# LiuTaowen-Tony/xKV

Measured on NVIDIA B200. Metric: KV GB/s compressed (prefill, xKV-4, Llama-3.1-8B 64K), higher is better.
Workload: dtype bf16

## Files before the change

include/xkv_b200.h:

```cpp
#ifndef XKV_B200_H_
#define XKV_B200_H_

#include <stddef.h>
#include <stdint.h>

#ifdef __cplusplus
extern "C" {
#endif

#if defined(__GNUC__)
#define XKV_API __attribute__((visibility("default")))
#else
#define XKV_API
#endif

#define XKV_MAX_GROUP_LAYERS 16
#define XKV_MAX_GEMM_PROBLEMS 16
#define XKV_MAX_BATCH 16
#define XKV_MAX_LAYER_MAPS 64

XKV_API const char* xkv_last_error(void);
XKV_API int xkv_version(void);
XKV_API int64_t xkv_launch_count(void);

XKV_API int xkv_pack_group(const void* const* layer_ptrs_host, int num_layers, int bs, int heads, int seq,
                   int head_dim, int64_t stride_b, int64_t stride_h, int64_t stride_s, void* X,
                   void* stream);
XKV_API int xkv_unpack_group(const void* X, int num_layers, int bs, int heads, int seq, int head_dim,
                     int64_t stride_b, int64_t stride_h, int64_t stride_s, void* const* layer_ptrs_host,
                     void* stream);

typedef struct xkv_gemm_problem {
  int32_t M, N, K;
  int32_t num_terms;
  int32_t a_mn_major;
  int32_t b_mn_major;
  const void* A[3];
  const void* B[3];
  int64_t lda, ldb;
  uint8_t term_a[6], term_b[6];
  void* D;
  int64_t ldd;
  int32_t out_bf16;
  int32_t out_transposed;
  int32_t sym_upper;
  int32_t split_k;
  int64_t split_stride;
  int32_t accum_phases;
  const int32_t* run_if;
  int32_t a_layers, b_layers, layer_cols;
  const void* A_layer[XKV_MAX_GROUP_LAYERS];
  const void* B_layer[XKV_MAX_GROUP_LAYERS];
} xkv_gemm_problem;
XKV_API int xkv_gemm_grouped(const xkv_gemm_problem* problems_host, int num_problems, void* stream);
XKV_API size_t xkv_gemm_problem_size(void);
XKV_API void xkv_gemm_set_gram_pair(int on);

XKV_API int xkv_reduce_slabs(const float* slabs, int num_slabs, int64_t slab_stride, int rows, int cols, int64_t ld,
                     int symmetrize, float* out, int64_t ld_out, void* stream);
XKV_API int xkv_reduce_slabs_batched(const float* const* slabs_host, float* const* out_host, int batch, int num_slabs,
                                     int64_t slab_stride, int rows, int cols, int64_t ld, int symmetrize,
                                     int64_t ld_out, void* stream);
XKV_API int xkv_split_bf16(const float* x, int rows, int cols, int64_t ld, void* hi, void* mid, void* lo,
                   int64_t ld_out, void* stream);
XKV_API int xkv_split_bf16_batched(const float* const* x_host, void* const* hi_host, void* const* mid_host,
                                   void* const* lo_host, int batch, int rows, int cols, int64_t ld, int64_t ld_out,
                                   void* stream);
XKV_API int xkv_symmetrize_split_bf16(const float* const* slabs_host, int batch, int num_slabs, int64_t slab_stride,
                                      int n, int64_t ld, void* const* hi_host, void* const* mid_host,
                                      void* const* lo_host, int64_t ld_out, void* stream);
XKV_API size_t xkv_gram_packed_elems(int n);
XKV_API int xkv_gram_pack_upper(const float* full, int n, int64_t ld, float* packed, void* stream);
XKV_API int xkv_gram_unpack_upper(const float* packed, int n, float* full, int64_t ld, void* stream);
XKV_API int xkv_fill_gaussian_bf16(void* out, int rows, int cols, int64_t ld, uint64_t seed, void* stream);
XKV_API int xkv_normalize_rows(float* const* Y_host, void* const* hi_host, void* const* mid_host,
                               void* const* lo_host, int batch, int rows, int cols, int64_t ld, int64_t ld_out,
                               void* stream);
XKV_API int xkv_shift_normalize_rows(float* const* Y_host, const float* const* Q_host, float* shift_dev,
                                     float* const* rdiag_host, int rdiag_first, void* const* hi_host,
                                     void* const* mid_host, void* const* lo_host, int batch, int rows, int cols,
                                     int64_t ld, int64_t ld_out, void* stream);
XKV_API int xkv_ritz_shift_update(float* const* rdiag_host, int batch, int rows, int tail_rows, float shift_scale,
                                  float* shift_dev, void* stream);
XKV_API int xkv_rdiag_update(float* const* rdiag_host, const float* const* Linv_host, int batch, int rows,
                             int64_t ld_linv, void* stream);
XKV_API int xkv_pass_flags(const float* const* Linv_host, int batch, int rows, int64_t ld_linv, float min_pivot,
                           int32_t* flags_dev, void* stream);
XKV_API void xkv_set_launch_predicate(const int32_t* flags_dev);
XKV_API int xkv_cholesky_inverse(float* const* S_host, float* const* Linv_host, int batch, int l, int64_t ld,
                                 float shift, float pivot_floor, void* stream);
XKV_API int xkv_cholesky_inverse_limbs(float* const* S_host, float* const* Linv_host, void* const* hi_host,
                                       void* const* mid_host, void* const* lo_host, int batch, int l, int64_t ld,
                                       int64_t ld_limb, float shift, float pivot_floor, void* stream);
XKV_API int xkv_jacobi_eigh(const float* const* T_host, float* const* evals_host, float* const* Wt_host, int count,
                            int W, int64_t ld, int64_t ld_w, int sweeps, void* stream);
XKV_API int xkv_convert_bf16(const float* src, int rows, int cols, int64_t ld, void* dst, int64_t ld_dst, void* dstT,
                             int64_t ld_dstT, void* stream);

XKV_API int xkv_sqrt_clamp(const float* in, float* out, int count, void* stream);

#define XKV_FACTORIZE_SIGMA_COUNT 128
// ... 62 lines not shown
```

xkv_b200/_lib.py:

```python
from __future__ import annotations

import ctypes as C
import os
from typing import Optional

_LIB_PATH = os.environ.get("XKV_B200_LIB") or os.path.join(os.path.dirname(os.path.abspath(__file__)), "libxkv_b200.so")
_lib: Optional[C.CDLL] = None

MAX_GROUP_LAYERS = 16
MAX_GEMM_PROBLEMS = 16
MAX_BATCH = 16
FACTORIZE_SIGMA_COUNT = 128


class XkvError(RuntimeError):
    """Raised when a C-ABI call returns a non-zero status (mirrors the reference's Python exceptions)."""


class GemmProblem(C.Structure):

    _fields_ = [
        ("M", C.c_int32),
        ("N", C.c_int32),
        ("K", C.c_int32),
        ("num_terms", C.c_int32),
        ("a_mn_major", C.c_int32),
        ("b_mn_major", C.c_int32),
        ("A", C.c_void_p * 3),
        ("B", C.c_void_p * 3),
        ("lda", C.c_int64),
        ("ldb", C.c_int64),
        ("term_a", C.c_uint8 * 6),
        ("term_b", C.c_uint8 * 6),
        ("D", C.c_void_p),
        ("ldd", C.c_int64),
        ("out_bf16", C.c_int32),
        ("out_transposed", C.c_int32),
        ("sym_upper", C.c_int32),
        ("split_k", C.c_int32),
        ("split_stride", C.c_int64),
        ("accum_phases", C.c_int32),
        ("run_if", C.c_void_p),
        ("a_layers", C.c_int32),
        ("b_layers", C.c_int32),
        ("layer_cols", C.c_int32),
        ("A_layer", C.c_void_p * MAX_GROUP_LAYERS),
        ("B_layer", C.c_void_p * MAX_GROUP_LAYERS),
    ]


class AppendProblem(C.Structure):

    _fields_ = [("x_new", C.c_void_p), ("V", C.c_void_p), ("a_out", C.c_void_p), ("ldx", C.c_int64), ("ldv", C.c_int64),
                ("lda", C.c_int64), ("n", C.c_int32), ("r", C.c_int32)]


_vp, _i, _i64, _f, _sz = C.c_void_p, C.c_int, C.c_int64, C.c_float, C.c_size_t
_pp = C.POINTER(C.c_void_p)
SIGNATURES = {
    "xkv_last_error": (C.c_char_p, []),
    "xkv_version": (_i, []),
    "xkv_launch_count": (_i64, []),
    "xkv_pack_group": (_i, [_pp, _i, _i, _i, _i, _i, _i64, _i64, _i64, _vp, _vp]),
    "xkv_unpack_group": (_i, [_vp, _i, _i, _i, _i, _i, _i64, _i64, _i64, _pp, _vp]),
    "xkv_gemm_grouped": (_i, [C.POINTER(GemmProblem), _i, _vp]),
    "xkv_reduce_slabs": (_i, [_vp, _i, _i64, _i, _i, _i64, _i, _vp, _i64, _vp]),
    "xkv_reduce_slabs_batched": (_i, [_pp, _pp, _i, _i, _i64, _i, _i, _i64, _i, _i64, _vp]),
    "xkv_symmetrize_split_bf16": (_i, [_pp, _i, _i, _i64, _i, _i64, _pp, _pp, _pp, _i64, _vp]),
    "xkv_split_bf16_batched": (_i, [_pp, _pp, _pp, _pp, _i, _i, _i, _i64, _i64, _vp]),
    "xkv_split_bf16": (_i, [_vp, _i, _i, _i64, _vp, _vp, _vp, _i64, _vp]),
    "xkv_gram_packed_elems": (_sz, [_i]),
    "xkv_gram_pack_upper": (_i, [_vp, _i, _i64, _vp, _vp]),
    "xkv_gram_unpack_upper": (_i, [_vp, _i, _vp, _i64, _vp]),
    "xkv_fill_gaussian_bf16": (_i, [_vp, _i, _i, _i64, C.c_uint64, _vp]),
    "xkv_normalize_rows": (_i, [_pp, _pp, _pp, _pp, _i, _i, _i, _i64, _i64, _vp]),
    "xkv_shift_normalize_rows": (_i, [_pp, _pp, _vp, _pp, _i, _pp, _pp, _pp, _i, _i, _i, _i64, _i64, _vp]),
    "xkv_ritz_shift_update": (_i, [_pp, _i, _i, _i, _f, _vp, _vp]),
    "xkv_rdiag_update": (_i, [_pp, _pp, _i, _i, _i64, _vp]),
    "xkv_pass_flags": (_i, [_pp, _i, _i, _i64, C.c_float, _vp, _vp]),
    "xkv_set_launch_predicate": (None, [_vp]),
    "xkv_cholesky_inverse": (_i, [_pp, _pp, _i, _i, _i64, _f, _f, _vp]),
    "xkv_cholesky_inverse_limbs": (_i, [_pp, _pp, _pp, _pp, _pp, _i, _i, _i64, _i64, _f, _f, _vp]),
    "xkv_jacobi_eigh": (_i, [_pp, _pp, _pp, _i, _i, _i64, _i64, _i, _vp]),
    "xkv_convert_bf16": (_i, [_vp, _i, _i, _i64, _vp, _i64, _vp, _i64, _vp]),
    "xkv_sqrt_clamp": (_i, [_vp, _vp, _i, _vp]),
    "xkv_factorize_workspace_bytes": (_sz, [_i, _i, _i, _i]),
    "xkv_decode_workspace_bytes": (_sz, [_i, _i, _i, _i]),
    "xkv_decode_attention": (_i, [_vp, _i, _i, _i, _vp, _i64, _i, _vp, _i64, _vp, _i64, _i, _vp, _i64, _i, _vp, _vp, _i64,
                                  _vp, _vp, _i, _i64, _i64, _f, _vp, _vp, _sz, _vp]),
    "xkv_decode_attention_lse": (_i, [_vp, _i, _i, _i, _vp, _i64, _i, _vp, _i64, _vp, _i64, _i, _vp, _i64, _i, _vp, _vp,
                                      _i64, _vp, _vp, _i, _i64, _i64, _f, _vp, _vp, _sz, _vp, _vp]),
    "xkv_decode_attention_multi": (_i, [_vp, _i, _i, _i, _i, _vp, _i64, _i, _vp, _i64, _vp, _i64, _i, _vp, _i64, _i, _vp,
                                        _vp, _i64, _vp, _vp, _i, _i64, _i64, _f, _vp, _vp, _sz, _vp, _vp]),
    "xkv_decode_absorbed_workspace_bytes": (_sz, [_i, _i, _i]),
# ... 43 lines not shown
```

xkv_b200/csrc/xkv_factorize.cu:

```cuda
#include <cuda_bf16.h>

#include <vector>

#include "xkv_host.h"

namespace xkv {

static inline size_t align_up(size_t x, size_t a) { return (x + a - 1) / a * a; }
static inline int round_up_int(int x, int k) { return (x + k - 1) / k * k; }

struct Bump {
  char* base;
  size_t off, cap;
  bool overflow;
  void* take(size_t bytes) {
    off = align_up(off, 1024);
    void* p = base ? base + off : nullptr;
    off += bytes;
    if (base && off > cap) overflow = true;
    return p;
  }
  float* f32(size_t n) { return static_cast<float*>(take(n * 4)); }
  void* bf16(size_t n) { return take(n * 2); }
};
// ... 252 lines not shown
    }
  }
  XKV_TRY(mark());
  if (phase == 1) return 0;

  float** cur = P.f_a;
  float** nxt = P.f_b;
  auto swap_bufs = [&]() {
    float** t = cur;
    cur = nxt;
    nxt = t;
  };
  auto cholqr = [&](bool shifted, bool track, bool final_call) -> int {
    const int first = shifted ? 1 : 0;
    for (int pp = first; pp <= first + 1; ++pp) {
      const bool cond = shifted && pp == 2;
      if (cond) {
        XKV_TRY(xkv_pass_flags(P.linv, B, l, l, kSecondPassMinPivot, P.pass_flags, stream));
        xkv_set_launch_predicate(P.pass_flags);
      }
      int rc = [&]() -> int {
        XKV_TRY(xkv_shift_normalize_rows(cur, (pp == first && shifted) ? nxt : nullptr, P.shift_dev,
                                         track ? P.rdiag : nullptr, pp == first, P.lh, P.lm, P.ll, B, l, n, nn, nn, stream));
        for (int b = 0; b < B; ++b) {
          xkv_gemm_problem p = problem(P.lh[b], P.lm[b], P.ll[b], nn, 0, P.lh[b], P.lm[b], P.ll[b], nn, 0, P.s_slabs[b],
                                       l, l, l, n, 6);
          p.sym_upper = 1;
          p.split_k = P.sk;
          p.split_stride = static_cast<long long>(l) * l;
          p.run_if = cond ? P.pass_flags + b : nullptr;
          ps.push_back(p);
        }
        XKV_TRY(run_gemms(ps, stream));
        XKV_TRY(xkv_reduce_slabs_batched(P.s_slabs, P.s_mat, B, P.sk, static_cast<long long>(l) * l, l, l, l, 1, l, stream));
        {
          void *h0[XKV_MAX_BATCH], *h1[XKV_MAX_BATCH], *h2[XKV_MAX_BATCH];
          for (int b = 0; b < B; ++b) h0[b] = P.linv_l[b][0], h1[b] = P.linv_l[b][1], h2[b] = P.linv_l[b][2];
          const float shift = kCholShift[pp];
          XKV_TRY(xkv_cholesky_inverse_limbs(P.s_mat, P.linv, h0, h1, h2, B, l, l, l, shift, kPivotFloor, stream));
          if (pp > 0) {
            XKV_TRY(xkv_pass_flags(P.linv, B, l, l, 2.f * shift, P.redo_flags, stream));
            xkv_set_launch_predicate(P.redo_flags);
            int rc2 = xkv_reduce_slabs_batched(P.s_slabs, P.s_mat, B, P.sk, static_cast<long long>(l) * l, l, l, l, 1, l, stream);
            if (!rc2)
              rc2 = xkv_cholesky_inverse_limbs(P.s_mat, P.linv, h0, h1, h2, B, l, l, l, kCholShift[0], kPivotFloor, stream);
            xkv_set_launch_predicate(cond ? P.pass_flags : nullptr);
            if (rc2) return rc2;
          }
        }
        if (track) XKV_TRY(xkv_rdiag_update(P.rdiag, P.linv, B, l, l, stream));
        for (int b = 0; b < B; ++b) {
          xkv_gemm_problem p = swap_roles(problem(P.linv_l[b][0], P.linv_l[b][1], P.linv_l[b][2], l, 0, P.lh[b], P.lm[b],
                                                  P.ll[b], nn, 1, cond ? cur[b] : nxt[b], nn, l, n, l, final_call ? 6 : 3));
          p.run_if = cond ? P.pass_flags + b : nullptr;
          ps.push_back(p);
        }
        XKV_TRY(run_gemms(ps, stream));
        return 0;
      }();
      if (cond) xkv_set_launch_predicate(nullptr);
      if (rc) return rc;
      if (!cond) swap_bufs();
    }
    return 0;
  };
  auto apply_gram = [&](int nterms) -> int {
    for (int b = 0; b < B; ++b)
      ps.push_back(swap_roles(problem(P.lh[b], P.lm[b], P.ll[b], nn, 0, P.g_limb[b][0], P.g_limb[b][1], P.g_limb[b][2], nn, 0,
                                      nxt[b], nn, l, n, n, nterms)));
    XKV_TRY(run_gemms(ps, stream));
    swap_bufs();
    return 0;
  };

  for (int b = 0; b < B; ++b) XKV_TRY(xkv_fill_gaussian_bf16(P.lh[b], l, n, nn, kSeed + 7919ull * b, stream));
  XKV_TRY(apply_gram(1));
  XKV_TRY(cholqr(false, false, false));
  XKV_TRY(mark());

  XKV_CHECK_CUDA(cudaMemsetAsync(P.shift_dev, 0, XKV_MAX_BATCH * sizeof(float), st));
  for (int it = 0; it < kPowerSteps; ++it) {
    XKV_TRY(xkv_split_bf16_batched(cur, P.lh, P.lm, nullptr, B, l, n, nn, nn, stream));
    XKV_TRY(apply_gram(3));
    if (it > 0) XKV_TRY(xkv_ritz_shift_update(P.rdiag, B, l, kShiftTail, kSpectralShift, P.shift_dev, stream));
    const bool last = it == kPowerSteps - 1;
    XKV_TRY(cholqr(it > 0, !last, last));
  }
  XKV_TRY(mark());

  {
    const int r0 = l - W, wl = r - r0;
    auto w0 = [&](int w) { return w == 0 ? r0 : 0; };
    XKV_TRY(xkv_split_bf16_batched(cur, P.lh, P.lm, P.ll, B, l, n, nn, nn, stream));
    for (int b = 0; b < B; ++b)
      for (int w = 0; w < 2; ++w)
        ps.push_back(swap_roles(problem(row_bf16(P.lh[b], w0(w), nn), row_bf16(P.lm[b], w0(w), nn),
                                        row_bf16(P.ll[b], w0(w), nn), nn, 0, P.g_limb[b][0], P.g_limb[b][1], P.g_limb[b][2],
                                        nn, 0, P.yw[b][w], nn, W, n, n, 6)));
    XKV_TRY(run_gemms(ps, stream));
    {
      const float* xs[2 * XKV_MAX_BATCH];
      void *h0[2 * XKV_MAX_BATCH], *h1[2 * XKV_MAX_BATCH], *h2[2 * XKV_MAX_BATCH];
      int cntw = 0;
      for (int b = 0; b < B; ++b)
        for (int w = 0; w < 2; ++w) {
          xs[cntw] = P.yw[b][w];
// ... 89 lines not shown
```

xkv_b200/csrc/xkv_gemm.cu:

```cuda
#include <cstdlib>

#include "xkv_common.cuh"
#include "xkv_host.h"

namespace xkv {

constexpr int BM = 128;
constexpr int BN = 256;
constexpr int BK = 64;
constexpr int STAGES = 4;
constexpr int A_TILE_BYTES = BM * BK * 2;
constexpr int B_TILE_BYTES = BN * BK * 2;
constexpr int STAGE_BYTES = A_TILE_BYTES + B_TILE_BYTES;
constexpr int CHUNK_BYTES = 64 * BK * 2;
constexpr int GEMM_THREADS = 192;
constexpr int TMEM_COLS = 256;
constexpr size_t GEMM_SMEM_BYTES = STAGES * STAGE_BYTES + 1024  + 256 ;

struct alignas(64) GemmProb {
  CUtensorMap a_map[3];
  CUtensorMap b_map[3];
  void* D;
  long long ldd;
  long long split_stride;
  int M, N, K;
  int nterms;
  int tiles_m, tiles_n, ntiles;
  int split_k, kblocks_per_split, nkb;
  int cta_begin;
  int bn;
  int na, nb;
  unsigned char la[3], lb[3];
  unsigned char sa[3], sb[3];
  int pstages;
  int out_bf16, out_transposed, sym_upper;
  unsigned char ta[6], tb[6];
  const int* run_if;
  int phases;
  int a_layers, a_layer_begin, b_layers, b_layer_begin, layer_cols;
};
struct GemmParams {
  int nprob;
  int pair_stages;
  GemmProb p[XKV_MAX_GEMM_PROBLEMS];
  CUtensorMap layer_maps[XKV_MAX_LAYER_MAPS];
};

__device__ __forceinline__ const CUtensorMap* layer_map(const GemmParams& P, int begin, int layers, int layer_cols, int col,
                                                        int& col_in_layer) {
  int li = col / layer_cols;
  li = li < layers ? li : layers - 1;
  col_in_layer = col - li * layer_cols;
  return &P.layer_maps[begin + li];
}

template <int A_MN, int B_MN>
__global__ void __launch_bounds__(GEMM_THREADS, 1) gemm_kernel(const __grid_constant__ GemmParams P) {
  extern __shared__ uint8_t smem_raw[];
  uint8_t* smem = reinterpret_cast<uint8_t*>((reinterpret_cast<uintptr_t>(smem_raw) + 1023) & ~uintptr_t(1023));
  uint64_t* full_bar = reinterpret_cast<uint64_t*>(smem + STAGES * STAGE_BYTES);
  uint64_t* empty_bar = full_bar + STAGES;
  uint64_t* tmem_full_bar = empty_bar + STAGES;
  uint64_t* tmem_empty_bar = tmem_full_bar + 2;
  uint32_t* tmem_slot = reinterpret_cast<uint32_t*>(tmem_empty_bar + 2);

  const int warp = threadIdx.x >> 5;
  const int lane = threadIdx.x & 31;

  int pi = 0;
  while (pi + 1 < P.nprob && static_cast<int>(blockIdx.x) >= P.p[pi + 1].cta_begin) ++pi;
  const GemmProb& pr = P.p[pi];
  if (pr.run_if != nullptr && *pr.run_if == 0) return;
  const int local = static_cast<int>(blockIdx.x) - pr.cta_begin;
  const int split = local / pr.ntiles;
  int t = local - split * pr.ntiles;
  int tm, tn;
  if (pr.sym_upper) {
    tm = 0;
    tn = 0;
    for (int i = 0; i < pr.tiles_m; ++i) {
      const int first = (i * BM) / BN;
      const int cnt = pr.tiles_n - first;
      if (t < cnt) {
        tm = i;
        tn = first + t;
        break;
      }
      t -= cnt;
    }
  } else {
    tm = t / pr.tiles_n;
    tn = t - tm * pr.tiles_n;
  }
  const int m0 = tm * BM;
  const int n0 = tn * BN;
  const int kb0 = split * pr.kblocks_per_split;
  const int kb1 = min(kb0 + pr.kblocks_per_split, pr.nkb);
  const int nk = max(kb1 - kb0, 0);
  const int niter = nk * pr.nterms;
  const int nph = max(1, min(pr.phases, nk));
  const uint32_t tmem_cols = nph > 1 ? 2 * TMEM_COLS : TMEM_COLS;

  if (warp == 0 && lane == 0) {
    for (int i = 0; i < STAGES; ++i) {
      mbar_init(&full_bar[i], 1);
      mbar_init(&empty_bar[i], 1);
    }
    mbar_init(&tmem_full_bar[0], 1);
    mbar_init(&tmem_full_bar[1], 1);
    mbar_init(&tmem_empty_bar[0], 4);
    mbar_init(&tmem_empty_bar[1], 4);
    mbar_fence_init();
    for (int i = 0; i < 3; ++i) {
      tma_prefetch_desc(&pr.a_map[i]);
      tma_prefetch_desc(&pr.b_map[i]);
    }
  }
  if (warp == 1) tmem_alloc(tmem_slot, tmem_cols);
  tc_fence_before();
  __syncthreads();
  tc_fence_after();
  const uint32_t tmem_base = *tmem_slot;

  if (warp == 0) {
    const CUtensorMap* a_chunk_map[BM / 64];
    int a_chunk_col[BM / 64];
    const CUtensorMap* b_chunk_map[BN / 64];
    int b_chunk_col[BN / 64];
#pragma unroll
    for (int c = 0; c < BM / 64; ++c) {
      a_chunk_col[c] = m0 + 64 * c;
      a_chunk_map[c] = (A_MN && pr.a_layers) ? layer_map(P, pr.a_layer_begin, pr.a_layers, pr.layer_cols, m0 + 64 * c, a_chunk_col[c]) : nullptr;
    }
#pragma unroll
    for (int c = 0; c < BN / 64; ++c) {
      b_chunk_col[c] = n0 + 64 * c;
      b_chunk_map[c] = (B_MN && pr.b_layers) ? layer_map(P, pr.b_layer_begin, pr.b_layers, pr.layer_cols, n0 + 64 * c, b_chunk_col[c]) : nullptr;
    }
    int ka_layer = 0, ka_col = 0, kb_layer = 0, kb_col = 0;
    if (!A_MN && pr.a_layers) {
      ka_layer = (kb0 * BK) / pr.layer_cols;
      ka_col = kb0 * BK - ka_layer * pr.layer_cols;
    }
    if (!B_MN && pr.b_layers) {
      kb_layer = (kb0 * BK) / pr.layer_cols;
      kb_col = kb0 * BK - kb_layer * pr.layer_cols;
    }
    if (elect_one()) {
      int s = 0, term = 0, kb = kb0;
      uint32_t ph = 0;
      for (int it = 0; it < niter; ++it) {
        const CUtensorMap* amap = &pr.a_map[pr.ta[term]];
        const CUtensorMap* bmap = &pr.b_map[pr.tb[term]];
        uint8_t* sA = smem + s * STAGE_BYTES;
        uint8_t* sB = sA + A_TILE_BYTES;
        mbar_wait(&empty_bar[s], ph ^ 1u);
        mbar_expect_tx(&full_bar[s], STAGE_BYTES);
        if (A_MN == 0) {
          if (pr.a_layers)
            tma_load_2d(sA, &P.layer_maps[pr.a_layer_begin + min(ka_layer, pr.a_layers - 1)], &full_bar[s],
                        ka_layer < pr.a_layers ? ka_col : pr.layer_cols, m0);
          else
            tma_load_2d(sA, amap, &full_bar[s], kb * BK, m0);
        } else {
#pragma unroll
          for (int c = 0; c < BM / 64; ++c)
            tma_load_2d(sA + c * CHUNK_BYTES, a_chunk_map[c] ? a_chunk_map[c] : amap, &full_bar[s], a_chunk_col[c], kb * BK);
        }
        if (B_MN == 0) {
          if (pr.b_layers)
            tma_load_2d(sB, &P.layer_maps[pr.b_layer_begin + min(kb_layer, pr.b_layers - 1)], &full_bar[s],
                        kb_layer < pr.b_layers ? kb_col : pr.layer_cols, n0);
          else
            tma_load_2d(sB, bmap, &full_bar[s], kb * BK, n0);
        } else {
#pragma unroll
          for (int c = 0; c < BN / 64; ++c)
            tma_load_2d(sB + c * CHUNK_BYTES, b_chunk_map[c] ? b_chunk_map[c] : bmap, &full_bar[s], b_chunk_col[c], kb * BK);
        }
        if (!A_MN && pr.a_layers && (ka_col += BK) >= pr.layer_cols) {
          ka_col -= pr.layer_cols;
          ++ka_layer;
        }
        if (!B_MN && pr.b_layers && (kb_col += BK) >= pr.layer_cols) {
          kb_col -= pr.layer_cols;
          ++kb_layer;
        }
        if (++term == pr.nterms) {
          term = 0;
          ++kb;
        }
        if (++s == STAGES) {
          s = 0;
          ph ^= 1u;
        }
      }
    }
    __syncwarp();
  } else if (warp == 1) {
    constexpr uint32_t idesc = umma_idesc_bf16(BM, BN, A_MN, B_MN);
    constexpr uint64_t kStageStep = STAGE_BYTES >> 4;
    constexpr uint64_t kAStep = (A_MN ? 2048 : 32) >> 4, kBStep = (B_MN ? 2048 : 32) >> 4;
    if (elect_one()) {
      const uint32_t a_base0 = smem_u32(smem);
      const uint64_t a_desc0 = A_MN ? umma_desc_sw128(a_base0, CHUNK_BYTES, 1024) : umma_desc_sw128(a_base0, 16, 1024);
      const uint64_t b_desc0 = B_MN ? umma_desc_sw128(a_base0 + A_TILE_BYTES, CHUNK_BYTES, 1024)
                                    : umma_desc_sw128(a_base0 + A_TILE_BYTES, 16, 1024);
      uint64_t a_desc = a_desc0, b_desc = b_desc0;
      int s = 0;
      uint32_t ph = 0;
      int it = 0;
      for (int phs = 0; phs < nph; ++phs) {
        const uint32_t acc = tmem_base + static_cast<uint32_t>(phs & 1) * TMEM_COLS;
        if (phs >= 2) {
          mbar_wait(&tmem_empty_bar[phs & 1], static_cast<uint32_t>(((phs >> 1) - 1) & 1));
          tc_fence_after();
        }
        const int it_end = (nph == 1) ? niter : static_cast<int>((static_cast<long long>(nk) * (phs + 1)) / nph) * pr.nterms;
        const int it_begin = it;
        for (; it < it_end; ++it) {
          mbar_wait(&full_bar[s], ph);
          tc_fence_after();
          umma_bf16_ss(acc, a_desc, b_desc, idesc, it > it_begin ? 1u : 0u);
          umma_bf16_ss(acc, a_desc + kAStep, b_desc + kBStep, idesc, 1u);
          umma_bf16_ss(acc, a_desc + 2 * kAStep, b_desc + 2 * kBStep, idesc, 1u);
          umma_bf16_ss(acc, a_desc + 3 * kAStep, b_desc + 3 * kBStep, idesc, 1u);
          umma_commit(&empty_bar[s]);
          a_desc += kStageStep;
          b_desc += kStageStep;
          if (++s == STAGES) {
            s = 0;
            ph ^= 1u;
            a_desc = a_desc0;
            b_desc = b_desc0;
          }
        }
        umma_commit(&tmem_full_bar[phs & 1]);
      }
    }
    __syncwarp();
  } else {
    const int q = warp & 3;
    const int row = m0 + q * 32 + lane;
    const bool row_ok = row < pr.M;
    float* outf = reinterpret_cast<float*>(pr.D) + static_cast<long long>(split) * pr.split_stride;
    __nv_bfloat16* outh = reinterpret_cast<__nv_bfloat16*>(pr.D) + static_cast<long long>(split) * pr.split_stride;
    const bool vec_ok = (pr.ldd % 8 == 0) && ((reinterpret_cast<uintptr_t>(pr.D) & 15) == 0) &&
                        ((pr.split_stride % 8) == 0);
#pragma unroll 1
    for (int phs = 0; phs < nph; ++phs) {
    float4 pre[8];
    auto prefetch = [&](int c) -> bool {
      const int col0 = n0 + c * 32;
      if (!(phs > 0 && row_ok && vec_ok && c < BN / 32 && col0 + 32 <= pr.N)) return false;
      const float4* src = reinterpret_cast<const float4*>(outf + static_cast<long long>(row) * pr.ldd + col0);
#pragma unroll
      for (int j = 0; j < 8; ++j) pre[j] = src[j];
      return true;
    };
    bool have_pre = prefetch(0);
    mbar_wait(&tmem_full_bar[phs & 1], static_cast<uint32_t>((phs >> 1) & 1));
    tc_fence_after();
    const uint32_t acc = tmem_base + static_cast<uint32_t>(phs & 1) * TMEM_COLS;
#pragma unroll 1
    for (int c = 0; c < BN / 32; ++c) {
      const int col0 = n0 + c * 32;
      if (col0 >= pr.N) break;
      uint32_t v[32];
      __syncwarp();
      if (niter > 0) {
        tmem_ld_32x32(acc + (static_cast<uint32_t>(q * 32) << 16) + static_cast<uint32_t>(c * 32), v);
        float4 cur[8];
        const bool have_cur = have_pre;
#pragma unroll
        for (int j = 0; j < 8; ++j) cur[j] = pre[j];
        have_pre = prefetch(c + 1);
        tmem_ld_wait();
        if (have_cur) {
#pragma unroll
          for (int j = 0; j < 8; ++j) {
            v[4 * j] = __float_as_uint(__uint_as_float(v[4 * j]) + cur[j].x);
            v[4 * j + 1] = __float_as_uint(__uint_as_float(v[4 * j + 1]) + cur[j].y);
            v[4 * j + 2] = __float_as_uint(__uint_as_float(v[4 * j + 2]) + cur[j].z);
            v[4 * j + 3] = __float_as_uint(__uint_as_float(v[4 * j + 3]) + cur[j].w);
          }
        } else if (phs > 0 && row_ok) {
          const float* src = outf + static_cast<long long>(row) * pr.ldd + col0;
#pragma unroll
          for (int j = 0; j < 32; ++j)
            if (col0 + j < pr.N) v[j] = __float_as_uint(__uint_as_float(v[j]) + src[j]);
        }
      } else {
#pragma unroll
        for (int j = 0; j < 32; ++j) v[j] = 0u;
      }
      const bool full = (col0 + 32 <= pr.N);
      if (!pr.out_transposed) {
        if (!row_ok) {
        } else if (!pr.out_bf16) {
          float* dst = outf + static_cast<long long>(row) * pr.ldd + col0;
          if (full && vec_ok) {
#pragma unroll
            for (int j = 0; j < 8; ++j)
              reinterpret_cast<uint4*>(dst)[j] = make_uint4(v[4 * j], v[4 * j + 1], v[4 * j + 2], v[4 * j + 3]);
          } else {
#pragma unroll
            for (int j = 0; j < 32; ++j)
              if (col0 + j < pr.N) dst[j] = __uint_as_float(v[j]);
          }
        } else {
          __nv_bfloat16* dst = outh + static_cast<long long>(row) * pr.ldd + col0;
          if (full && vec_ok) {
#pragma unroll
            for (int j = 0; j < 4; ++j) {
              uint4 w;
              w.x = pack_bf16x2(__uint_as_float(v[8 * j + 0]), __uint_as_float(v[8 * j + 1]));
              w.y = pack_bf16x2(__uint_as_float(v[8 * j + 2]), __uint_as_float(v[8 * j + 3]));
              w.z = pack_bf16x2(__uint_as_float(v[8 * j + 4]), __uint_as_float(v[8 * j + 5]));
              w.w = pack_bf16x2(__uint_as_float(v[8 * j + 6]), __uint_as_float(v[8 * j + 7]));
              reinterpret_cast<uint4*>(dst)[j] = w;
            }
          } else {
#pragma unroll
            for (int j = 0; j < 32; ++j)
              if (col0 + j < pr.N) dst[j] = __float2bfloat16_rn(__uint_as_float(v[j]));
          }
        }
      } else {
        if (!pr.out_bf16) {
#pragma unroll
          for (int j = 0; j < 32; ++j)
            if (row_ok && col0 + j < pr.N)
              outf[static_cast<long long>(col0 + j) * pr.ldd + row] = __uint_as_float(v[j]);
        } else {
#pragma unroll
          for (int j = 0; j < 32; ++j)
            if (row_ok && col0 + j < pr.N)
              outh[static_cast<long long>(col0 + j) * pr.ldd + row] = __float2bfloat16_rn(__uint_as_float(v[j]));
        }
// ... 10 lines not shown
  tc_fence_before();
  __syncthreads();
  if (warp == 1) {
    tc_fence_after();
    tmem_dealloc(tmem_base, tmem_cols);
  }
}

constexpr int PG_BM = 256;
constexpr int PG_STAGES = 6;
constexpr int PG_MAX_STAGES = 7;
constexpr int PG_A_BYTES = BM * BK * 2;
constexpr int PG_B_BYTES = (BN / 2) * BK * 2;
constexpr int PG_STAGE_BYTES = PG_A_BYTES + PG_B_BYTES;
constexpr size_t pg_smem_bytes(int stages) { return static_cast<size_t>(stages) * PG_STAGE_BYTES + 1024  + 256 ; }

template <int A_MN, int B_MN>
__global__ void __launch_bounds__(GEMM_THREADS, 1) gemm_pair_kernel(const __grid_constant__ GemmParams P) {
  extern __shared__ uint8_t smem_raw[];
  uint8_t* smem = reinterpret_cast<uint8_t*>((reinterpret_cast<uintptr_t>(smem_raw) + 1023) & ~uintptr_t(1023));
  uint64_t* full_bar = reinterpret_cast<uint64_t*>(smem + P.pair_stages * PG_STAGE_BYTES);
  uint64_t* empty_bar = full_bar + PG_MAX_STAGES;
  uint64_t* tmem_full_bar = empty_bar + PG_MAX_STAGES;
  uint64_t* tmem_empty_bar = tmem_full_bar + 2;
  uint32_t* tmem_slot = reinterpret_cast<uint32_t*>(tmem_empty_bar + 2);

  const int warp = threadIdx.x >> 5;
  const int lane = threadIdx.x & 31;
  const int crank = static_cast<int>(cluster_ctarank());
  const bool leader = crank == 0;

  int pi = 0;
  while (pi + 1 < P.nprob && static_cast<int>(blockIdx.x) >= P.p[pi + 1].cta_begin) ++pi;
  const GemmProb& pr = P.p[pi];
  if (pr.run_if != nullptr && *pr.run_if == 0) return;
  const int bn = pr.bn;
  const int nstages = pr.pstages;
  const int na = pr.na;
  const uint32_t stage_bytes = static_cast<uint32_t>(pr.na + pr.nb) * PG_A_BYTES;
  const int local = (static_cast<int>(blockIdx.x) - pr.cta_begin) >> 1;
  const int split = local / pr.ntiles;
  int t = local - split * pr.ntiles;
  int tm = 0, tn = 0;
  if (pr.sym_upper) {
    for (int i = 0; i < pr.tiles_m; ++i) {
      const int cnt = pr.tiles_n - i;
      if (t < cnt) {
        tm = i;
        tn = i + t;
        break;
      }
      t -= cnt;
    }
  } else {
    tm = t / pr.tiles_n;
    tn = t - tm * pr.tiles_n;
  }
  const int m0 = tm * PG_BM + crank * BM;
  const int n0 = tn * bn;
  const int nb0 = n0 + crank * (bn >> 1);
  const int n_end = min(pr.N, n0 + bn);
  const int kb0 = split * pr.kblocks_per_split;
  const int kb1 = min(kb0 + pr.kblocks_per_split, pr.nkb);
  const int nk = max(kb1 - kb0, 0);
  const int niter = nk * pr.nterms;
  const int nph = max(1, min(pr.phases, nk));
  const uint32_t tmem_cols = nph > 1 ? 2 * TMEM_COLS : TMEM_COLS;
  const uint32_t b_bytes = B_MN ? static_cast<uint32_t>(PG_B_BYTES) : static_cast<uint32_t>(bn >> 1) * (BK * 2);

  if (warp == 0 && lane == 0) {
    for (int i = 0; i < nstages; ++i) {
      mbar_init(&full_bar[i], 1);
      mbar_init(&empty_bar[i], 1);
    }
    mbar_init(&tmem_full_bar[0], 1);
    mbar_init(&tmem_full_bar[1], 1);
    mbar_init(&tmem_empty_bar[0], 8);
    mbar_init(&tmem_empty_bar[1], 8);
    mbar_fence_init();
    tma_prefetch_desc(&pr.a_map[pr.ta[0]]);
    tma_prefetch_desc(&pr.b_map[pr.tb[0]]);
  }
  if (warp == 1) tmem_alloc_pair(tmem_slot, tmem_cols);
  tc_fence_before();
  __syncthreads();
  cluster_sync_all();
  tc_fence_after();
  const uint32_t tmem_base = *tmem_slot;

  if (warp == 0) {
    const CUtensorMap* a_chunk_map[2];
    const CUtensorMap* b_chunk_map[2];
    int a_chunk_col[2], b_chunk_col[2];
#pragma unroll
    for (int c = 0; c < 2; ++c) {
      a_chunk_col[c] = m0 + 64 * c;
      a_chunk_map[c] = (A_MN && pr.a_layers) ? layer_map(P, pr.a_layer_begin, pr.a_layers, pr.layer_cols, m0 + 64 * c, a_chunk_col[c]) : nullptr;
      b_chunk_col[c] = nb0 + 64 * c;
      b_chunk_map[c] = (B_MN && pr.b_layers) ? layer_map(P, pr.b_layer_begin, pr.b_layers, pr.layer_cols, nb0 + 64 * c, b_chunk_col[c]) : nullptr;
    }
    int ka_layer = 0, ka_col = 0, kb_layer = 0, kb_col = 0;
    if (!A_MN && pr.a_layers) {
      ka_layer = (kb0 * BK) / pr.layer_cols;
      ka_col = kb0 * BK - ka_layer * pr.layer_cols;
    }
    if (!B_MN && pr.b_layers) {
      kb_layer = (kb0 * BK) / pr.layer_cols;
      kb_col = kb0 * BK - kb_layer * pr.layer_cols;
    }
    if (elect_one()) {
      int s = 0;
      uint32_t ph = 0;
      const uint32_t full0 = cluster_map_shared(smem_u32(&full_bar[0]), 0);
      const uint32_t tx = 2u * (static_cast<uint32_t>(pr.na) * PG_A_BYTES + static_cast<uint32_t>(pr.nb) * b_bytes);
      for (int kb = kb0; kb < kb1; ++kb) {
        uint8_t* sA = smem + s * stage_bytes;
// ... 177 lines not shown
                w.w = pack_bf16x2(__uint_as_float(v[8 * j + 6]), __uint_as_float(v[8 * j + 7]));
                reinterpret_cast<uint4*>(dst)[j] = w;
              }
            } else {
#pragma unroll
              for (int j = 0; j < 32; ++j)
                if (col0 + j < n_end) dst[j] = __float2bfloat16_rn(__uint_as_float(v[j]));
            }
          }
        } else {
          if (!pr.out_bf16) {
#pragma unroll
            for (int j = 0; j < 32; ++j)
              if (row_ok && col0 + j < n_end)
                outf[static_cast<long long>(col0 + j) * pr.ldd + row] = __uint_as_float(v[j]);
          } else {
#pragma unroll
            for (int j = 0; j < 32; ++j)
              if (row_ok && col0 + j < n_end)
                outh[static_cast<long long>(col0 + j) * pr.ldd + row] = __float2bfloat16_rn(__uint_as_float(v[j]));
          }
        }
      }
      if (phs + 2 < nph) {
        tc_fence_before();
        __syncwarp();
        if (lane == 0) mbar_arrive_cluster(tempty0 + static_cast<uint32_t>((phs & 1) * 8));
      }
    }
  }

  tc_fence_before();
  __syncthreads();
  cluster_sync_all();
  if (warp == 1) {
    tc_fence_after();
    tmem_dealloc_pair(tmem_base, tmem_cols);
  }
}

static bool g_gram_pair = true;

static int pair_bn(const xkv_gemm_problem& p) {
  if (!g_gram_pair) return 0;
  const int rem = p.M % PG_BM;
  if (!(p.M >= 2048 || rem == 0 || rem > BM)) return 0;
  if (p.sym_upper) return (p.a_mn_major && p.b_mn_major && p.M == p.N) ? BN : 0;
  if (p.b_mn_major) return BN;
  const int ntn = (p.N + BN - 1) / BN;
  const int w = (p.N + ntn - 1) / ntn;
  return (w + 15) & ~15;
}

static int build_problem(const xkv_gemm_problem& in, GemmProb& out, int& cta_cursor, GemmParams& params, int& map_cursor,
                         int pair_n = 0) {
  const bool pair = pair_n > 0;
  const int bn = pair ? pair_n : BN;
  XKV_REQUIRE(in.M > 0 && in.N > 0 && in.K > 0, "gemm: empty problem M=%d N=%d K=%d", in.M, in.N, in.K);
  XKV_REQUIRE(in.num_terms >= 1 && in.num_terms <= 6, "gemm: num_terms=%d out of range", in.num_terms);
  XKV_REQUIRE(in.lda % 8 == 0 && in.ldb % 8 == 0, "gemm: lda/ldb must be multiples of 8 elements");
  XKV_REQUIRE(in.split_k >= 1, "gemm: split_k must be >= 1");
  XKV_REQUIRE(in.D != nullptr, "gemm: null output");
  std::memset(&out, 0, sizeof(out));
  bool used_a[3] = {false, false, false}, used_b[3] = {false, false, false};
  for (int t = 0; t < in.num_terms; ++t) {
    XKV_REQUIRE(in.term_a[t] < 3 && in.term_b[t] < 3, "gemm: limb index out of range");
    used_a[in.term_a[t]] = true;
    used_b[in.term_b[t]] = true;
    out.ta[t] = in.term_a[t];
    out.tb[t] = in.term_b[t];
  }
  XKV_REQUIRE(in.a_layers >= 0 && in.a_layers <= XKV_MAX_GROUP_LAYERS && in.b_layers >= 0 && in.b_layers <= XKV_MAX_GROUP_LAYERS,
              "gemm: at most %d layers per operand", XKV_MAX_GROUP_LAYERS);
  if (in.a_layers > 0 || in.b_layers > 0) {
    XKV_REQUIRE(in.num_terms == 1, "gemm: layered operands take one term");
    XKV_REQUIRE(in.layer_cols > 0 && in.layer_cols % 64 == 0, "gemm: layer_cols=%d must be a positive multiple of 64", in.layer_cols);
  }
  for (int side = 0; side < 2; ++side) {
    const int layers = side == 0 ? in.a_layers : in.b_layers;
    if (layers == 0) continue;
    const void* const* ptrs = side == 0 ? in.A_layer : in.B_layer;
    const bool mn = side == 0 ? in.a_mn_major != 0 : in.b_mn_major != 0;
    const long long ld = side == 0 ? in.lda : in.ldb;
    const int other = side == 0 ? in.M : in.N;
    if (side == 1 && in.a_layers == in.b_layers && in.a_mn_major && in.b_mn_major && in.lda == in.ldb &&
        std::memcmp(in.A_layer, in.B_layer, sizeof(void*) * layers) == 0) {
      out.b_layer_begin = out.a_layer_begin;
      continue;
    }
    (side == 0 ? out.a_layer_begin : out.b_layer_begin) = map_cursor;
    for (int i = 0; i < layers; ++i) {
      XKV_REQUIRE(ptrs[i] != nullptr && (reinterpret_cast<uintptr_t>(ptrs[i]) & 15) == 0, "gemm: layer %d null or unaligned", i);
      XKV_REQUIRE(map_cursor < XKV_MAX_LAYER_MAPS, "gemm: more than %d layer matrices in one launch", XKV_MAX_LAYER_MAPS);
      int rc;
      if (!mn)
        rc = encode_tmap_2d_bf16(&params.layer_maps[map_cursor++], ptrs[i], in.layer_cols, other, ld, BK,
                                 side == 0 ? BM : (pair ? bn / 2 : BN));
      else
        rc = encode_tmap_2d_bf16(&params.layer_maps[map_cursor++], ptrs[i], in.layer_cols, in.K, ld, 64, BK);
      if (rc) return rc;
    }
  }
  out.a_layers = in.a_layers;
  out.b_layers = in.b_layers;
  out.layer_cols = in.layer_cols;
  XKV_REQUIRE(in.a_layers == 0 || (in.a_mn_major ? in.M : in.K) <= in.a_layers * in.layer_cols, "gemm: layered A narrower than the problem");
  XKV_REQUIRE(in.b_layers == 0 || (in.b_mn_major ? in.N : in.K) <= in.b_layers * in.layer_cols, "gemm: layered B narrower than the problem");
  for (int i = 0; i < 3; ++i) {
    const void* a = in.a_layers > 0 ? in.A_layer[0] : (used_a[i] ? in.A[i] : in.A[in.term_a[0]]);
    const void* b = in.b_layers > 0 ? in.B_layer[0] : (used_b[i] ? in.B[i] : in.B[in.term_b[0]]);
    XKV_REQUIRE(a != nullptr && b != nullptr, "gemm: null operand limb %d", i);
    XKV_REQUIRE((reinterpret_cast<uintptr_t>(a) & 15) == 0 && (reinterpret_cast<uintptr_t>(b) & 15) == 0,
                "gemm: operands must be 16-byte aligned");
    int rc = 0;
    if (in.a_layers > 0)
      out.a_map[i] = params.layer_maps[out.a_layer_begin];
    else if (!in.a_mn_major)
      rc = encode_tmap_2d_bf16(&out.a_map[i], a, in.K, in.M, in.lda, BK, BM);
    else
      rc = encode_tmap_2d_bf16(&out.a_map[i], a, in.M, in.K, in.lda, 64, BK);
    if (rc) return rc;
    if (in.b_layers > 0)
      out.b_map[i] = params.layer_maps[out.b_layer_begin];
    else if (!in.b_mn_major)
      rc = encode_tmap_2d_bf16(&out.b_map[i], b, in.K, in.N, in.ldb, BK, pair ? bn / 2 : BN);
    else
      rc = encode_tmap_2d_bf16(&out.b_map[i], b, in.N, in.K, in.ldb, 64, BK);
    if (rc) return rc;
  }
  out.D = in.D;
  out.ldd = in.ldd;
  out.split_stride = in.split_stride;
  out.M = in.M;
  out.N = in.N;
  out.K = in.K;
  out.nterms = in.num_terms;
  const int bm = pair ? PG_BM : BM;
  out.bn = bn;
  out.tiles_m = (in.M + bm - 1) / bm;
  out.tiles_n = (in.N + bn - 1) / bn;
  out.sym_upper = in.sym_upper ? 1 : 0;
  if (out.sym_upper) {
    int cnt = 0;
    for (int i = 0; i < out.tiles_m; ++i) cnt += out.tiles_n - (i * bm) / bn;
    out.ntiles = cnt;
  } else {
    out.ntiles = out.tiles_m * out.tiles_n;
  }
  for (int i = 0; i < 3; ++i) {
    if (used_a[i]) {
      out.sa[i] = static_cast<unsigned char>(out.na);
      out.la[out.na++] = static_cast<unsigned char>(i);
    }
    if (used_b[i]) {
      out.sb[i] = static_cast<unsigned char>(out.nb);
      out.lb[out.nb++] = static_cast<unsigned char>(i);
    }
  }
  out.nkb = (in.K + BK - 1) / BK;
  out.split_k = in.split_k;
  out.kblocks_per_split = (out.nkb + in.split_k - 1) / in.split_k;
  out.out_bf16 = in.out_bf16 ? 1 : 0;
  out.out_transposed = in.out_transposed ? 1 : 0;
  out.run_if = in.run_if;
  out.phases = in.accum_phases > 1 ? in.accum_phases : 1;
  XKV_REQUIRE(out.phases == 1 || (!in.out_bf16 && !in.out_transposed),
              "gemm: accum_phases > 1 needs a plain fp32 output");
  out.cta_begin = cta_cursor;
  cta_cursor += out.ntiles * out.split_k * (pair ? 2 : 1);
  return 0;
}

bool& gemm_low_priority() {
  static thread_local bool low = false;
  return low;
}

template <int A_MN, int B_MN>
static int launch_pair_variant(GemmParams& params, int grid, cudaStream_t stream) {
  auto kern = gemm_pair_kernel<A_MN, B_MN>;
  static PerDevice<bool> configured;
  if (!configured()) {
    XKV_CHECK_CUDA(cudaFuncSetAttribute(kern, cudaFuncAttributeMaxDynamicSharedMemorySize,
                                        static_cast<int>(pg_smem_bytes(PG_MAX_STAGES))));
    configured() = true;
  }
  params.pair_stages = PG_STAGES;
  for (int i = 0; i < params.nprob; ++i) {
    const int stage = (params.p[i].na + params.p[i].nb) * PG_A_BYTES;
    const int st = params.pair_stages * PG_STAGE_BYTES / stage;
    params.p[i].pstages = st > PG_MAX_STAGES ? PG_MAX_STAGES : st;
  }
  cudaLaunchConfig_t cfg;
  std::memset(&cfg, 0, sizeof(cfg));
  cfg.gridDim = dim3(grid, 1, 1);
  cfg.blockDim = dim3(GEMM_THREADS, 1, 1);
  cfg.dynamicSmemBytes = pg_smem_bytes(params.pair_stages);
  cfg.stream = stream;
  cudaLaunchAttribute attr[2];
  attr[0].id = cudaLaunchAttributeClusterDimension;
  attr[0].val.clusterDim.x = 2;
  attr[0].val.clusterDim.y = 1;
  attr[0].val.clusterDim.z = 1;
  cfg.numAttrs = 1;
  if (gemm_low_priority()) {
    attr[1].id = cudaLaunchAttributePriority;
    attr[1].val.priority = 0;
    cfg.numAttrs = 2;
  }
  cfg.attrs = attr;
  XKV_CHECK_CUDA(cudaLaunchKernelEx(&cfg, kern, params));
  XKV_LAUNCHED();
  return 0;
}

template <int A_MN, int B_MN>
static int launch_variant(const GemmParams& params, int grid, cudaStream_t stream) {
  auto kern = gemm_kernel<A_MN, B_MN>;
  static PerDevice<bool> configured;
  if (!configured()) {
    XKV_CHECK_CUDA(cudaFuncSetAttribute(kern, cudaFuncAttributeMaxDynamicSharedMemorySize,
                                        static_cast<int>(GEMM_SMEM_BYTES)));
// ... 57 lines not shown
```

Before: 243.8.

## Skip zero K-blocks for lower-triangular B and pack two splits per CTA

```diff
diff --git a/include/xkv_b200.h b/include/xkv_b200.h
--- a/include/xkv_b200.h
+++ b/include/xkv_b200.h
@@ -47,6 +47,7 @@
   int32_t split_k;
   int64_t split_stride;
   int32_t accum_phases;
+  int32_t b_lower_tri_k;
   const int32_t* run_if;
   int32_t a_layers, b_layers, layer_cols;
   const void* A_layer[XKV_MAX_GROUP_LAYERS];
diff --git a/xkv_b200/_lib.py b/xkv_b200/_lib.py
--- a/xkv_b200/_lib.py
+++ b/xkv_b200/_lib.py
@@ -40,6 +40,7 @@
         ("split_k", C.c_int32),
         ("split_stride", C.c_int64),
         ("accum_phases", C.c_int32),
+        ("b_lower_tri_k", C.c_int32),
         ("run_if", C.c_void_p),
         ("a_layers", C.c_int32),
         ("b_layers", C.c_int32),
diff --git a/xkv_b200/csrc/xkv_factorize.cu b/xkv_b200/csrc/xkv_factorize.cu
--- a/xkv_b200/csrc/xkv_factorize.cu
+++ b/xkv_b200/csrc/xkv_factorize.cu
@@ -328,6 +328,7 @@
         for (int b = 0; b < B; ++b) {
           xkv_gemm_problem p = swap_roles(problem(P.linv_l[b][0], P.linv_l[b][1], P.linv_l[b][2], l, 0, P.lh[b], P.lm[b],
                                                   P.ll[b], nn, 1, cond ? cur[b] : nxt[b], nn, l, n, l, final_call ? 6 : 3));
+          p.b_lower_tri_k = 1;
           p.run_if = cond ? P.pass_flags + b : nullptr;
           ps.push_back(p);
         }
diff --git a/xkv_b200/csrc/xkv_gemm.cu b/xkv_b200/csrc/xkv_gemm.cu
--- a/xkv_b200/csrc/xkv_gemm.cu
+++ b/xkv_b200/csrc/xkv_gemm.cu
@@ -29,6 +29,8 @@
   int split_k, kblocks_per_split, nkb;
   int cta_begin;
   int bn;
+  int b_tri;
+  int spc;
   int na, nb;
   unsigned char la[3], lb[3];
   unsigned char sa[3], sb[3];
@@ -71,15 +73,17 @@
   while (pi + 1 < P.nprob && static_cast<int>(blockIdx.x) >= P.p[pi + 1].cta_begin) ++pi;
   const GemmProb& pr = P.p[pi];
   if (pr.run_if != nullptr && *pr.run_if == 0) return;
+  const int bn = pr.bn;
   const int local = static_cast<int>(blockIdx.x) - pr.cta_begin;
-  const int split = local / pr.ntiles;
-  int t = local - split * pr.ntiles;
+  const int group = local / pr.ntiles;
+  const int split = group * pr.spc;
+  int t = local - group * pr.ntiles;
   int tm, tn;
   if (pr.sym_upper) {
     tm = 0;
     tn = 0;
     for (int i = 0; i < pr.tiles_m; ++i) {
-      const int first = (i * BM) / BN;
+      const int first = (i * BM) / bn;
       const int cnt = pr.tiles_n - first;
       if (t < cnt) {
         tm = i;
@@ -88,17 +92,21 @@
       }
       t -= cnt;
     }
+  } else if (pr.b_tri) {
+    tn = pr.tiles_n - 1 - t / pr.tiles_m;
+    tm = t - (pr.tiles_n - 1 - tn) * pr.tiles_m;
   } else {
     tm = t / pr.tiles_n;
     tn = t - tm * pr.tiles_n;
   }
   const int m0 = tm * BM;
-  const int n0 = tn * BN;
+  const int n0 = tn * bn;
   const int kb0 = split * pr.kblocks_per_split;
-  const int kb1 = min(kb0 + pr.kblocks_per_split, pr.nkb);
+  int kb1 = min(kb0 + pr.spc * pr.kblocks_per_split, pr.nkb);
+  if (pr.b_tri) kb1 = min(kb1, (min(pr.N, n0 + bn) + BK - 1) / BK);
   const int nk = max(kb1 - kb0, 0);
   const int niter = nk * pr.nterms;
-  const int nph = max(1, min(pr.phases, nk));
+  const int nph = pr.spc > 1 ? pr.spc : max(1, min(pr.phases, nk));
   const uint32_t tmem_cols = nph > 1 ? 2 * TMEM_COLS : TMEM_COLS;
 
   if (warp == 0 && lane == 0) {
@@ -149,13 +157,14 @@
     if (elect_one()) {
       int s = 0, term = 0, kb = kb0;
       uint32_t ph = 0;
+      const uint32_t tx = static_cast<uint32_t>(A_TILE_BYTES + bn * BK * 2);
       for (int it = 0; it < niter; ++it) {
         const CUtensorMap* amap = &pr.a_map[pr.ta[term]];
         const CUtensorMap* bmap = &pr.b_map[pr.tb[term]];
         uint8_t* sA = smem + s * STAGE_BYTES;
         uint8_t* sB = sA + A_TILE_BYTES;
         mbar_wait(&empty_bar[s], ph ^ 1u);
-        mbar_expect_tx(&full_bar[s], STAGE_BYTES);
+        mbar_expect_tx(&full_bar[s], tx);
         if (A_MN == 0) {
           if (pr.a_layers)
             tma_load_2d(sA, &P.layer_maps[pr.a_layer_begin + min(ka_layer, pr.a_layers - 1)], &full_bar[s],
@@ -176,7 +185,8 @@
         } else {
 #pragma unroll
           for (int c = 0; c < BN / 64; ++c)
-            tma_load_2d(sB + c * CHUNK_BYTES, b_chunk_map[c] ? b_chunk_map[c] : bmap, &full_bar[s], b_chunk_col[c], kb * BK);
+            if (c * 64 < bn)
+              tma_load_2d(sB + c * CHUNK_BYTES, b_chunk_map[c] ? b_chunk_map[c] : bmap, &full_bar[s], b_chunk_col[c], kb * BK);
         }
         if (!A_MN && pr.a_layers && (ka_col += BK) >= pr.layer_cols) {
           ka_col -= pr.layer_cols;
@@ -198,7 +208,7 @@
     }
     __syncwarp();
   } else if (warp == 1) {
-    constexpr uint32_t idesc = umma_idesc_bf16(BM, BN, A_MN, B_MN);
+    const uint32_t idesc = umma_idesc_bf16(BM, 0, A_MN, B_MN) | (static_cast<uint32_t>(bn >> 3) << 17);
     constexpr uint64_t kStageStep = STAGE_BYTES >> 4;
     constexpr uint64_t kAStep = (A_MN ? 2048 : 32) >> 4, kBStep = (B_MN ? 2048 : 32) >> 4;
     if (elect_one()) {
@@ -243,16 +253,18 @@
     const int q = warp & 3;
     const int row = m0 + q * 32 + lane;
     const bool row_ok = row < pr.M;
-    float* outf = reinterpret_cast<float*>(pr.D) + static_cast<long long>(split) * pr.split_stride;
-    __nv_bfloat16* outh = reinterpret_cast<__nv_bfloat16*>(pr.D) + static_cast<long long>(split) * pr.split_stride;
     const bool vec_ok = (pr.ldd % 8 == 0) && ((reinterpret_cast<uintptr_t>(pr.D) & 15) == 0) &&
                         ((pr.split_stride % 8) == 0);
+    const bool add = pr.spc == 1;
 #pragma unroll 1
     for (int phs = 0; phs < nph; ++phs) {
+    const long long slab = split + (add ? 0 : phs);
+    float* outf = reinterpret_cast<float*>(pr.D) + slab * pr.split_stride;
+    __nv_bfloat16* outh = reinterpret_cast<__nv_bfloat16*>(pr.D) + slab * pr.split_stride;
     float4 pre[8];
     auto prefetch = [&](int c) -> bool {
       const int col0 = n0 + c * 32;
-      if (!(phs > 0 && row_ok && vec_ok && c < BN / 32 && col0 + 32 <= pr.N)) return false;
+      if (!(add && phs > 0 && row_ok && vec_ok && c < bn / 32 && col0 + 32 <= pr.N)) return false;
       const float4* src = reinterpret_cast<const float4*>(outf + static_cast<long long>(row) * pr.ldd + col0);
 #pragma unroll
       for (int j = 0; j < 8; ++j) pre[j] = src[j];
@@ -263,7 +275,7 @@
     tc_fence_after();
     const uint32_t acc = tmem_base + static_cast<uint32_t>(phs & 1) * TMEM_COLS;
 #pragma unroll 1
-    for (int c = 0; c < BN / 32; ++c) {
+    for (int c = 0; c < bn / 32; ++c) {
       const int col0 = n0 + c * 32;
       if (col0 >= pr.N) break;
       uint32_t v[32];
@@ -284,7 +296,7 @@
             v[4 * j + 2] = __float_as_uint(__uint_as_float(v[4 * j + 2]) + cur[j].z);
             v[4 * j + 3] = __float_as_uint(__uint_as_float(v[4 * j + 3]) + cur[j].w);
           }
-        } else if (phs > 0 && row_ok) {
+        } else if (add && phs > 0 && row_ok) {
           const float* src = outf + static_cast<long long>(row) * pr.ldd + col0;
 #pragma unroll
           for (int j = 0; j < 32; ++j)
@@ -401,6 +413,9 @@
       }
       t -= cnt;
     }
+  } else if (pr.b_tri) {
+    tn = pr.tiles_n - 1 - t / pr.tiles_m;
+    tm = t - (pr.tiles_n - 1 - tn) * pr.tiles_m;
   } else {
     tm = t / pr.tiles_n;
     tn = t - tm * pr.tiles_n;
@@ -410,7 +425,8 @@
   const int nb0 = n0 + crank * (bn >> 1);
   const int n_end = min(pr.N, n0 + bn);
   const int kb0 = split * pr.kblocks_per_split;
-  const int kb1 = min(kb0 + pr.kblocks_per_split, pr.nkb);
+  int kb1 = min(kb0 + pr.kblocks_per_split, pr.nkb);
+  if (pr.b_tri) kb1 = min(kb1, (n_end + BK - 1) / BK);
   const int nk = max(kb1 - kb0, 0);
   const int niter = nk * pr.nterms;
   const int nph = max(1, min(pr.phases, nk));
@@ -694,11 +710,17 @@
   return (w + 15) & ~15;
 }
 
+constexpr int kSymTileN = 128;
+constexpr int kSplitsPerCta = 2;
+static int single_bn(const xkv_gemm_problem& p) { return p.sym_upper ? kSymTileN : BN; }
+
 static int build_problem(const xkv_gemm_problem& in, GemmProb& out, int& cta_cursor, GemmParams& params, int& map_cursor,
                          int pair_n = 0) {
   const bool pair = pair_n > 0;
-  const int bn = pair ? pair_n : BN;
+  const int bn = pair ? pair_n : single_bn(in);
   XKV_REQUIRE(in.M > 0 && in.N > 0 && in.K > 0, "gemm: empty problem M=%d N=%d K=%d", in.M, in.N, in.K);
+  XKV_REQUIRE(!in.b_lower_tri_k || (!in.b_mn_major && in.split_k == 1),
+              "gemm: b_lower_tri_k needs a K-major B and split_k = 1");
   XKV_REQUIRE(in.num_terms >= 1 && in.num_terms <= 6, "gemm: num_terms=%d out of range", in.num_terms);
   XKV_REQUIRE(in.lda % 8 == 0 && in.ldb % 8 == 0, "gemm: lda/ldb must be multiples of 8 elements");
   XKV_REQUIRE(in.split_k >= 1, "gemm: split_k must be >= 1");
@@ -737,7 +759,7 @@
       int rc;
       if (!mn)
         rc = encode_tmap_2d_bf16(&params.layer_maps[map_cursor++], ptrs[i], in.layer_cols, other, ld, BK,
-                                 side == 0 ? BM : (pair ? bn / 2 : BN));
+                                 side == 0 ? BM : (pair ? bn / 2 : bn));
       else
         rc = encode_tmap_2d_bf16(&params.layer_maps[map_cursor++], ptrs[i], in.layer_cols, in.K, ld, 64, BK);
       if (rc) return rc;
@@ -765,7 +787,7 @@
     if (in.b_layers > 0)
       out.b_map[i] = params.layer_maps[out.b_layer_begin];
     else if (!in.b_mn_major)
-      rc = encode_tmap_2d_bf16(&out.b_map[i], b, in.K, in.N, in.ldb, BK, pair ? bn / 2 : BN);
+      rc = encode_tmap_2d_bf16(&out.b_map[i], b, in.K, in.N, in.ldb, BK, pair ? bn / 2 : bn);
     else
       rc = encode_tmap_2d_bf16(&out.b_map[i], b, in.N, in.K, in.ldb, 64, BK);
     if (rc) return rc;
@@ -782,6 +804,7 @@
   out.tiles_m = (in.M + bm - 1) / bm;
   out.tiles_n = (in.N + bn - 1) / bn;
   out.sym_upper = in.sym_upper ? 1 : 0;
+  out.b_tri = in.b_lower_tri_k ? 1 : 0;
   if (out.sym_upper) {
     int cnt = 0;
     for (int i = 0; i < out.tiles_m; ++i) cnt += out.tiles_n - (i * bm) / bn;
@@ -808,8 +831,12 @@
   out.phases = in.accum_phases > 1 ? in.accum_phases : 1;
   XKV_REQUIRE(out.phases == 1 || (!in.out_bf16 && !in.out_transposed),
               "gemm: accum_phases > 1 needs a plain fp32 output");
+  out.spc = 1;
+  if (!pair && out.sym_upper && out.phases == 1 && in.split_k % kSplitsPerCta == 0 &&
+      out.kblocks_per_split * in.split_k == out.nkb)
+    out.spc = kSplitsPerCta;
   out.cta_begin = cta_cursor;
-  cta_cursor += out.ntiles * out.split_k * (pair ? 2 : 1);
+  cta_cursor += out.ntiles * (out.split_k / out.spc) * (pair ? 2 : 1);
   return 0;
 }
 
```

Result: no change. 247.5, median of 6 (+1.5%).
